# YonghaoHe/LFD-A-Light-and-Fast-Detector

Hardware: AMD Instinct MI355X
Metric: images/sec WIDERFACE-S 1920x1080 bs=8 end-to-end inference, LFD.precision='fp32_storage' (raw logits within 1e-4 of fp32: inside north_star's 1e-3; the 'fp16' mode, sigma 2.5e-3, under fp16_mode) (higher is better)
Workload: dtype f16

## Files before the change

### include/lfd_hip.h

```cpp
#ifndef LFD_HIP_H_
#define LFD_HIP_H_

#include <stddef.h>
#include <stdint.h>

#ifdef __cplusplus
extern "C" {
#endif

#define LFD_HIP_ABI_VERSION 3
#define LFD_MAX_LEVELS 8

typedef void* lfd_stream_t;

#if defined(LFD_BUILDING)
#define LFD_API __attribute__((visibility("default")))
#else
#define LFD_API
#endif

enum lfd_status {
  LFD_OK = 0,
  LFD_ERR_INVALID_ARGUMENT = -1,
  LFD_ERR_WORKSPACE_TOO_SMALL = -2,
// ... 332 lines not shown
  const float* b0;
  const void* w1;
  const float* b1;
  void* gn_sums;
  const void* gn_in_sums;
  const float* gn_in_gamma;
  const float* gn_in_beta;
  float* f_out0;
  float* f_out1;
  const float* scale1;
  int64_t in_plane_halfs;
  int32_t pixels, pad_;
} lfd_pl_head_level_t;
LFD_API int lfd_pl_head_levels(const lfd_pl_head_desc_t* desc, const lfd_pl_head_level_t* levels, int32_t num_levels,
                               const void* zeros, lfd_stream_t stream);

LFD_API int lfd_stem_conv_f16(const void* in, int32_t in_format, int32_t n, int32_t h, int32_t w,
                              int32_t channels, const void* w1_packed, const float* b1,
                              const void* w2_packed, const float* b2, void* out, lfd_stream_t stream);

LFD_API int lfd_stem_gray_f16(const void* in, int32_t in_format, int32_t n, int32_t h, int32_t w, int32_t channels,
                              const void* w1_packed, const float* b1, const void* w2_packed, const float* b2, void* out,
                              lfd_stream_t stream);
LFD_API int lfd_pl_stem_gray_pair(const void* in, int32_t in_format, int32_t n, int32_t h, int32_t w, int32_t channels,
                                  const void* w1_packed, const float* b1, const void* w2_packed, const float* b2, void* out,
                                  int64_t out_plane_halfs, lfd_stream_t stream);

LFD_API int lfd_stem_faster_fused_f16(const void* in, int32_t in_format, int32_t n, int32_t h, int32_t w,
                                      int32_t channels, const void* w1_packed, const float* b1,
                                      const void* w2_packed, const float* b2, const void* w3_packed,
// ... 468 lines not shown
```

### lfd-a-light-and-fast-detector_amd/csrc/planes_head.hip

```cpp
#include "planes_impl.h"

namespace pl {

struct PhLevel {
  const void* in;
  long in_plane;
  float* out;
  const half8* w0;
  const float* b0;
  const half8* w1;
  const float* b1;
  unsigned long long* gn_out;
  const unsigned long long* gn_in;
  const float* gamma;
  const float* beta;
  float* f_out0;
  float* f_out1;
  const float* scale1;
  int P, tiles_per_img, tile_start, pad_;
};
struct PhArgs {
  PhLevel lv[LFD_MAX_LEVELS];
  const _Float16* zeros;
  long w_plane0, w_plane1;
// ... 21 lines not shown
  static_assert(LDS_BYTES <= 80 * 1024, "two workgroups per CU");
};

__device__ __forceinline__ double wave_sum(double v) {
#pragma unroll
  for (int d = 32; d >= 1; d >>= 1) v += __shfl_xor(v, d);
  return v;
}

#ifdef LFD_PL_TIMING
#define PH_T(i) do { if (blockIdx.x == PL_DBG_BLOCK && threadIdx.x == 0 && dbg_it < 8) g_pl_dbg[dbg_it * 16 + (i)] = __builtin_readcyclecounter(); } while (0)
#else
#define PH_T(i)
#endif

template <int MODE, int CIN, int NSLAB>
__global__ __launch_bounds__(256, 2) void k_pl_head(PhArgs a) {
  using C = PhCfg<MODE, CIN, NSLAB>;
  extern __shared__ __attribute__((aligned(16))) char smem[];
  const int lane = threadIdx.x & 63;
  const int wave = __builtin_amdgcn_readfirstlane((int)(threadIdx.x >> 6));
  const int h = lane >> 5, pix = lane & 31;
  constexpr int PT = MODE == 2 ? 1 : 2;
  const int slab = MODE == 2 ? (wave % NSLAB) : wave;
  const int pt0 = MODE == 2 ? (wave / NSLAB) : 0;
  const bool mfma_wave = MODE != 2 || wave < 2 * NSLAB;

  const int nblk = gridDim.x;
  const int xcd = blockIdx.x & 7, bix = blockIdx.x >> 3;
  const int per_xcd = (a.ntiles + 7) / 8;
  const int t_begin = xcd * per_xcd;
  const int t_end = (t_begin + per_xcd) < a.ntiles ? (t_begin + per_xcd) : a.ntiles;
  const int wgs_xcd = (nblk + 7 - xcd) / 8;
#ifdef PH_STRIDED
  const int t_step = wgs_xcd;
  const int t_first = t_begin + bix, t_last = t_end;
#else
  const int t_step = 1;
  const int chunk = (t_end - t_begin + wgs_xcd - 1) / (wgs_xcd > 0 ? wgs_xcd : 1);
  const int t_first = t_begin + bix * chunk;
  const int t_last = (t_first + chunk) < t_end ? (t_first + chunk) : t_end;
#endif
  int lstart[LFD_MAX_LEVELS];
#pragma unroll
  for (int i = 0; i < LFD_MAX_LEVELS; ++i) lstart[i] = i < a.n_levels ? a.lv[i].tile_start : 0x7fffffff;
  auto level_of = [&](int t) {
    int l = 0;
#pragma unroll
    for (int i = 1; i < LFD_MAX_LEVELS; ++i) l += (t >= lstart[i]) ? 1 : 0;
    return l;
  };

  auto with_level = [&](int l, auto&& f) {
    static_for([&](auto ic) {
      constexpr int i = decltype(ic)::value;
      if (l == i) f(a.lv[i]);
    }, std::make_integer_sequence<int, LFD_MAX_LEVELS>{});
// ... 113 lines not shown
  int buf = 0;
  bool first = true;
  if (t < t_last) issue_in(t, 0);

  for (; t < t_last; t += t_step, ++dbg_it) {
    PH_T(0);
    const int l = level_of(t);
    const bool new_level = l != cur_l;
    if (new_level) with_level(l, [&](const PhLevel& v) { lv = v; });
    const int rel = t - lv.tile_start;
    const int n = rel / lv.tiles_per_img;
    const int j = rel - n * lv.tiles_per_img;
    const int p0 = j * C::TPX;
    const bool has_next = t + t_step < t_last;

    if (first) asm volatile("s_waitcnt vmcnt(0)" ::: "memory");
    else if constexpr (MODE != 2) asm volatile("s_waitcnt vmcnt(8)" ::: "memory");
    else {
      switch (n_st) {
        case 0: asm volatile("s_waitcnt vmcnt(0)" ::: "memory"); break;
        case 1: asm volatile("s_waitcnt vmcnt(1)" ::: "memory"); break;
        case 2: asm volatile("s_waitcnt vmcnt(2)" ::: "memory"); break;
        case 3: asm volatile("s_waitcnt vmcnt(3)" ::: "memory"); break;
        case 4: asm volatile("s_waitcnt vmcnt(4)" ::: "memory"); break;
        case 5: asm volatile("s_waitcnt vmcnt(5)" ::: "memory"); break;
        case 6: asm volatile("s_waitcnt vmcnt(6)" ::: "memory"); break;
        case 7: asm volatile("s_waitcnt vmcnt(7)" ::: "memory"); break;
        case 8: asm volatile("s_waitcnt vmcnt(8)" ::: "memory"); break;
        case 9: asm volatile("s_waitcnt vmcnt(9)" ::: "memory"); break;
        case 10: asm volatile("s_waitcnt vmcnt(10)" ::: "memory"); break;
        case 11: asm volatile("s_waitcnt vmcnt(11)" ::: "memory"); break;
// ... 6 lines not shown
    }
    first = false;
    PH_T(1);
    block_barrier();
    PH_T(2);
    if constexpr (PLANES_IN && C::NBUF == 2) {
      if (has_next) issue_in(t + t_step, buf ^ 1);
    }

    if (new_level) {
      cur_l = l;
      const half8* ws = lv.w0 + ((size_t)slab * C::NK0) * 64 + lane;
#pragma unroll
      for (int k = 0; k < C::NK0; ++k) {
        w0h[k] = ws[(size_t)k * 64];
        w0l[k] = ws[a.w_plane0 + (size_t)k * 64];
      }
      if constexpr (MODE == 0) {
        const half8* w1s = lv.w1 + ((size_t)slab * 8) * 64 + lane;
#pragma unroll
        for (int k = 0; k < 8; ++k) {
          w1h[k] = w1s[(size_t)k * 64];
          w1l[k] = w1s[a.w_plane1 + (size_t)k * 64];
        }
      }
      if (threadIdx.x < 128) {
        sbias[threadIdx.x] = (MODE == 2 && (int)threadIdx.x >= NSLAB * 32) ? 0.f : lv.b0[threadIdx.x];
        if constexpr (MODE == 0) sbias[128 + threadIdx.x] = lv.b1[threadIdx.x];
      }
      if constexpr (MODE == 2) {
        n_st = 0;
        if (mfma_wave) {
#pragma unroll
          for (int i = 0; i < 16; ++i) n_st += (slab * 32 + 8 * (i >> 2) + (i & 3) < a.f_c0 + a.f_c1) ? 1 : 0;
        }
      }
      gnin_key = -1;
      block_barrier();
    }

    const char* op = smem + C::OP_OFF;
    if constexpr (!PLANES_IN) {
      const int pj = (int)threadIdx.x & 31, gi = pj >> 1;
      if (gnin_key != n) {
        gnin_key = n;
        long long s = 0, q = 0;
#pragma unroll
        for (int r = 0; r < kGnRep; ++r) {
          s += (long long)lv.gn_in[(((size_t)r * a.N + n) * 16 + gi) * 2];
          q += (long long)lv.gn_in[(((size_t)r * a.N + n) * 16 + gi) * 2 + 1];
        }
        const double cnt = (double)lv.P * 8.0;
        const double m = (double)s / kGnFix / cnt;
        double var = (double)q / kGnFix / cnt - m * m;
        var = var > 0. ? var : 0.;
        const float rstd = (float)(1. / sqrt(var + (double)a.eps)), mean = (float)m;
#pragma unroll
        for (int e = 0; e < 4; ++e) {
          gn_a[e] = rstd * lv.gamma[pj * 4 + e];
          gn_b[e] = lv.beta[pj * 4 + e] - mean * gn_a[e];
        }
      }
      const char* raw = smem + C::IN_OFF;
      char* opw = smem + C::OP_OFF;
#pragma unroll
      for (int r = 0; r < 8; ++r) {
        const int p = ((int)threadIdx.x >> 5) + 8 * r;
        const float4 v = *reinterpret_cast<const float4*>(raw + p * 512 + pj * 16);
        const float y0 = fmaxf(fmaf(v.x, gn_a[0], gn_b[0]), 0.f), y1 = fmaxf(fmaf(v.y, gn_a[1], gn_b[1]), 0.f);
        const float y2 = fmaxf(fmaf(v.z, gn_a[2], gn_b[2]), 0.f), y3 = fmaxf(fmaf(v.w, gn_a[3], gn_b[3]), 0.f);
        uint2 oh, ol;
        split2(y0, y1, oh.x, ol.x);
        split2(y2, y3, oh.y, ol.y);
        const int o = p * 256 + ((gi ^ (p & 15)) * 16) + (pj & 1) * 8;
        *reinterpret_cast<uint2*>(opw + o) = oh;
        *reinterpret_cast<uint2*>(opw + C::OP_PLANE + o) = ol;
      }
      PH_T(3);
      block_barrier();
      PH_T(4);
      if (has_next) issue_in(t + t_step, 0);
      PH_T(5);
// ... 46 lines not shown

    if constexpr (MODE == 0) {
      const char* xb = smem + C::IN_OFF + buf * 2 * C::IN_PLANE;
      init_acc(sbias + slab * 32 + 4 * h);
      contract([&](int q, int pt) { return xb + xi[pt] + (((2 * q) ^ xikey) << 4); }, C::IN_PLANE, w0h, w0l, std::integral_constant<int, C::NK0>{});
      char* mid = smem + C::OP_OFF;
#pragma unroll
      for (int pt = 0; pt < 2; ++pt) {
        const int pb = pt * 32 + pix;
#pragma unroll
        for (int g = 0; g < 4; ++g) {
          float y[4];
#pragma unroll
          for (int e = 0; e < 4; ++e) {
            y[e] = comb(am[pt][4 * g + e], ac[pt][4 * g + e]);
            if (a.relu0) y[e] = fmaxf(y[e], 0.f);
          }
          uint2 vh, vl;
          split2(y[0], y[1], vh.x, vl.x);
          split2(y[2], y[3], vh.y, vl.y);
          const int o = pb * 256 + (((slab * 4 + g) ^ (pb & 15)) * 16) + 8 * h;
          *reinterpret_cast<uint2*>(mid + o) = vh;
          *reinterpret_cast<uint2*>(mid + C::OP_PLANE + o) = vl;
        }
      }
      block_barrier();
      if constexpr (C::NBUF == 1) {
        if (has_next) issue_in(t + t_step, 0);
      }
      init_acc(sbias + 128 + slab * 32 + 4 * h);
      contract([&](int q, int pt) { return op_addr(op, q, pt); }, C::OP_PLANE, w1h, w1l, std::integral_constant<int, 8>{});
// ... 2 lines not shown
      init_acc(sbias + slab * 32 + 4 * h);
      contract([&](int q, int pt) { return xb + xi[pt] + (((2 * q) ^ xikey) << 4); }, C::IN_PLANE, w0h, w0l, std::integral_constant<int, C::NK0>{});
    } else {
      if (mfma_wave) {
        init_acc(sbias + slab * 32 + 4 * h);
        contract([&](int q, int pt) { return op_addr(op, q, pt); }, C::OP_PLANE, w0h, w0l, std::integral_constant<int, 8>{});
      }
    }

    PH_T(6);
    if constexpr (MODE != 2) {
      if (n != gn_n || l != gn_l) {
        gn_flush();
        gn_n = n; gn_l = l; gn_dst = lv.gn_out;
      }
      float* trash = reinterpret_cast<float*>(const_cast<_Float16*>(a.zeros) + 1024) + (threadIdx.x & 127) * 4;
      float* obase = lv.out + ((size_t)n * lv.P + p0) * 128 + slab * 32 + 4 * h;
#pragma unroll
      for (int pt = 0; pt < 2; ++pt) {
        const int px = pt * 32 + pix;
        const bool ok = p0 + px < lv.P;
        float* orow = obase + (size_t)px * 128;
#pragma unroll
        for (int g = 0; g < 4; ++g) {
          float4 v;
          v.x = comb(am[pt][4 * g + 0], ac[pt][4 * g + 0]);
          v.y = comb(am[pt][4 * g + 1], ac[pt][4 * g + 1]);
          v.z = comb(am[pt][4 * g + 2], ac[pt][4 * g + 2]);
          v.w = comb(am[pt][4 * g + 3], ac[pt][4 * g + 3]);
          *reinterpret_cast<float4*>(ok ? orow + 8 * g : trash) = v;
          if (ok) {
            const float s = (v.x + v.y) + (v.z + v.w);
            const float q = fmaf(v.x, v.x, fmaf(v.y, v.y, fmaf(v.z, v.z, v.w * v.w)));
            gs[g] += (double)s;
            gq[g] += (double)q;
          }
        }
      }
    } else {
      if (mfma_wave) {
        const float sc1 = lv.scale1 ? *lv.scale1 : 1.f;
        const int ctot = a.f_c0 + a.f_c1;
        float* trash = reinterpret_cast<float*>(const_cast<_Float16*>(a.zeros) + 1024) + (threadIdx.x & 127);
        const int px = p0 + pt0 * 32 + pix;
        const bool in_img = px < lv.P;
        const size_t pixi = in_img ? (size_t)px : 0;
        float* q0 = lv.f_out0 + (size_t)n * a.f_img0 + pixi * a.f_c0;
        float* q1 = lv.f_out1 + (size_t)n * a.f_img1 + pixi * a.f_c1 - a.f_c0;
#pragma unroll
        for (int g = 0; g < 4; ++g)
#pragma unroll
          for (int e = 0; e < 4; ++e) {
            if (slab * 32 + 8 * g + e < ctot) {
              const int co = slab * 32 + 8 * g + 4 * h + e;
              const float y = comb(am[0][4 * g + e], ac[0][4 * g + e]);
              const bool first_out = co < a.f_c0;
              float* dst = (in_img && co < ctot) ? (first_out ? q0 : q1) + co : trash;
              *dst = first_out ? y : y * sc1;
            }
          }
      }
    }
    if constexpr (PLANES_IN && C::NBUF == 2) buf ^= 1;
    PH_T(7);
  }
  gn_flush();
}

template <int NSLAB>
__global__ __launch_bounds__(256, 2) void k_pl_head_out(PhArgs a) {
  constexpr int TPX = 64, OP_PLANE = TPX * 256, BIAS_OFF = 4 * OP_PLANE;
  extern __shared__ __attribute__((aligned(16))) char smem[];
  const int lane = threadIdx.x & 63;
  const int wave = __builtin_amdgcn_readfirstlane((int)(threadIdx.x >> 6));
  const int h = lane >> 5, pix = lane & 31;
  const int slab = wave % NSLAB, pt0 = wave / NSLAB;
  const bool mfma_wave = wave < 2 * NSLAB;
  const int pj = (int)threadIdx.x & 31, gi = pj >> 1, prow = (int)threadIdx.x >> 5;
  const int nblk = gridDim.x;
  const int xcd = blockIdx.x & 7, bix = blockIdx.x >> 3;
  const int per_xcd = (a.ntiles + 7) / 8;
// ... 448 lines not shown
  static unsigned long long attr_done_mask = 0;
  const int attr_done_dev = lfd_device_ordinal();
  if (LFD_ONCE_PER_DEVICE(attr_done_mask, attr_done_dev)) {
    if (hipFuncSetAttribute(reinterpret_cast<const void*>(kern), hipFuncAttributeMaxDynamicSharedMemorySize, C::LDS_BYTES) != hipSuccess)
      return LFD_ERR_LAUNCH_FAILED;
    LFD_DONE_ON_DEVICE(attr_done_mask, attr_done_dev);
  }
  int blocks = 512;
  if (blocks > 8 * ((a.ntiles + 7) / 8)) blocks = 8 * ((a.ntiles + 7) / 8);
  if (blocks < 1) blocks = 1;
  hipLaunchKernelGGL(kern, dim3(blocks), dim3(256), C::LDS_BYTES, st, a);
  LFD_CHECK_LAUNCH();
  return LFD_OK;
}

}

#ifdef LFD_PL_TIMING
extern "C" __attribute__((visibility("default"))) int lfd_debug_pl_head_timing(unsigned long long* host_out) {
  return (int)hipMemcpyFromSymbol(host_out, HIP_SYMBOL(pl::g_pl_dbg), sizeof(unsigned long long) * 136);
}
#endif

extern "C" int lfd_pl_head_levels(const lfd_pl_head_desc_t* d, const lfd_pl_head_level_t* levels, int32_t num_levels, const void* zeros,
                                  lfd_stream_t stream) {
  hipStream_t st = reinterpret_cast<hipStream_t>(stream);
  if (!d || !levels || !zeros || num_levels < 1 || num_levels > LFD_MAX_LEVELS || d->n < 1) return LFD_ERR_INVALID_ARGUMENT;
  if (d->mode < 0 || d->mode > 3) return LFD_ERR_INVALID_ARGUMENT;
  if (d->mode == 0 && d->cin != 64 && d->cin != 128) return LFD_ERR_UNSUPPORTED;
  if (d->mode == 2 && (d->f_c0 < 0 || d->f_c1 < 0 || d->f_c0 + d->f_c1 < 1 || d->f_c0 + d->f_c1 > 64)) return LFD_ERR_UNSUPPORTED;
  pl::PhArgs a{};
  a.zeros = (const _Float16*)zeros;
  a.n_levels = num_levels; a.N = d->n; a.relu0 = d->relu0; a.eps = d->gn_in_eps;
  a.f_c0 = d->f_c0; a.f_c1 = d->f_c1; a.f_img0 = d->f_image_stride0; a.f_img1 = d->f_image_stride1;
  const int nslab0 = d->mode == 2 ? (d->f_c0 + d->f_c1 + 31) / 32 : 4;
  const int nk0 = (d->mode == 0 ? d->cin : 128) / 16;
  a.w_plane0 = (long)nslab0 * nk0 * 64;
  a.w_plane1 = 4L * 8 * 64;
  for (int i = 0; i < num_levels; ++i) {
    const lfd_pl_head_level_t& s = levels[i];
    if (!s.in || !s.w0 || !s.b0 || s.pixels < 1) return LFD_ERR_INVALID_ARGUMENT;
    if (!lfd_aligned16(s.in) || !lfd_aligned16(s.out) || (s.in_plane_halfs & 7)) return LFD_ERR_INVALID_ARGUMENT;
    if (d->mode == 0 && (!s.w1 || !s.b1)) return LFD_ERR_INVALID_ARGUMENT;
    if (d->mode != 2 && (!s.out || !s.gn_sums)) return LFD_ERR_INVALID_ARGUMENT;
    if ((d->mode == 1 || d->mode == 2) && (!s.gn_in_sums || !s.gn_in_gamma || !s.gn_in_beta)) return LFD_ERR_INVALID_ARGUMENT;
    if (d->mode == 2 && ((d->f_c0 > 0 && !s.f_out0) || (d->f_c1 > 0 && !s.f_out1))) return LFD_ERR_INVALID_ARGUMENT;
    pl::PhLevel& l = a.lv[i];
    l.in = s.in; l.in_plane = s.in_plane_halfs; l.out = (float*)s.out;
    l.w0 = (const half8*)s.w0; l.b0 = s.b0; l.w1 = (const half8*)s.w1; l.b1 = s.b1;
    l.gn_out = (unsigned long long*)s.gn_sums; l.gn_in = (const unsigned long long*)s.gn_in_sums;
    l.gamma = s.gn_in_gamma; l.beta = s.gn_in_beta;
    l.f_out0 = s.f_out0; l.f_out1 = s.f_out1; l.scale1 = s.scale1;
    l.P = s.pixels;
  }
  if (d->mode == 0) return d->cin == 64 ? pl::launch_pl_head<0, 64, 4>(a, st) : pl::launch_pl_head<0, 128, 4>(a, st);
  if (d->mode == 3) return pl::launch_pl_head<3, 128, 4>(a, st);
  if (d->mode == 1) return lfd_tune(LFD_TUNE_PL_HEAD_ROLES) != 0 ? pl::launch_pl_head_b2(a, st) : pl::launch_pl_head<1, 128, 4>(a, st);
  if (lfd_tune(LFD_TUNE_PL_HEAD_OUT_REGS) != 0) return nslab0 == 1 ? pl::launch_pl_head_out<1>(a, st) : pl::launch_pl_head_out<2>(a, st);
  return nslab0 == 1 ? pl::launch_pl_head<2, 128, 1>(a, st) : pl::launch_pl_head<2, 128, 2>(a, st);
}
```

### lfd-a-light-and-fast-detector_amd/lfd_amd/_lib.py

```python
import ctypes as C
import os

_HERE = os.path.dirname(os.path.abspath(__file__))
LIB_PATH = os.environ.get('LFD_HIP_LIB') or os.path.join(_HERE, 'liblfd_hip.so')
MAX_LEVELS = 8
F32, F16 = 0, 1

_lib = None


class DetectDesc(C.Structure):
    _fields_ = [('num_levels', C.c_int32),
                ('level_h', C.c_int32 * MAX_LEVELS), ('level_w', C.c_int32 * MAX_LEVELS),
                ('level_stride', C.c_int32 * MAX_LEVELS),
                ('level_range_lo', C.c_float * MAX_LEVELS), ('level_range_hi', C.c_float * MAX_LEVELS),
                ('num_classes', C.c_int32), ('num_cls_channels', C.c_int32),
                ('score_mode', C.c_int32), ('decode_mode', C.c_int32),
                ('class_agnostic', C.c_int32), ('max_candidates', C.c_int32),
                ('score_thr', C.c_float), ('iou_thr', C.c_float)]


class DetectExt(C.Structure):
    _fields_ = [('pre_nms_limit', C.c_int32), ('post_nms_limit', C.c_int32)]

# ... 57 lines not shown
class PlLevel(C.Structure):
    _fields_ = [(k, C.c_void_p) for k in ('in_', 'out', 'w_packed', 'bias', 'tail_w_packed', 'tail_bias', 'gn_sums', 'gn_in_sums',
                                          'gn_in_gamma', 'gn_in_beta', 'f_out0', 'f_out1', 'scale1')] + \
               [('h', C.c_int32), ('w', C.c_int32), ('in_plane_halfs', C.c_int64), ('out_plane_halfs', C.c_int64)]


class PlHeadDesc(C.Structure):
    _fields_ = [('mode', C.c_int32), ('n', C.c_int32), ('cin', C.c_int32), ('relu0', C.c_int32), ('f_c0', C.c_int32), ('f_c1', C.c_int32),
                ('gn_in_eps', C.c_float), ('pad_', C.c_int32), ('f_image_stride0', C.c_int64), ('f_image_stride1', C.c_int64)]


class PlHeadLevel(C.Structure):
    _fields_ = [(k, C.c_void_p) for k in ('in_', 'out', 'w0', 'b0', 'w1', 'b1', 'gn_sums', 'gn_in_sums', 'gn_in_gamma', 'gn_in_beta',
                                          'f_out0', 'f_out1', 'scale1')] + \
               [('in_plane_halfs', C.c_int64), ('pixels', C.c_int32), ('pad_', C.c_int32)]


PL_GN_REPLICAS = 8
ABI_VERSION = 3
HEAD_FOLDED_HALFS = 4 * 9 * 64 * 8
HEAD_TOWER1_GROUP_HALFS = 8 * 64 * 8


class AssignDesc(C.Structure):
    _fields_ = [('n', C.c_int32), ('num_levels', C.c_int32),
                ('level_h', C.c_int32 * MAX_LEVELS), ('level_w', C.c_int32 * MAX_LEVELS), ('stride', C.c_int32 * MAX_LEVELS),
                ('reg_lo', C.c_int32 * MAX_LEVELS), ('reg_hi', C.c_int32 * MAX_LEVELS),
                ('gray_lo', C.c_int32 * MAX_LEVELS), ('gray_hi', C.c_int32 * MAX_LEVELS),
                ('total_points', C.c_int32), ('num_classes', C.c_int32),
                ('assign_mode', C.c_int32), ('independent', C.c_int32)]
# ... 235 lines not shown
    'lfd_conv_packed_weight_halfs': (_SZ, [_I32, _I32, _I32]),
    'lfd_conv2d_nhwc_f16': (C.c_int, [C.POINTER(ConvDesc), _P, _P, _P, _P, _P, _P, _P, _P, _P]),
    'lfd_fasterblock_fused_f16': (C.c_int, [_I32, _I32, _I32, _P, _P, _P, _P, _P, _P, _P, _P]),
    'lfd_fasterblock128_fused_f16': (C.c_int, [_I32, _I32, _I32, _P, _P, _P, _P, _P, _P, _P]),
    'lfd_downblock_fused_f16': (C.c_int, [_I32, _I32, _I32, _P, _P, _P, _P, _P, _P, _P, _P, _P, _P]),
    'lfd_conv2d_nhwc_f16_acc32': (C.c_int, [C.POINTER(ConvDesc), _P, _P, _P, _P, _P, _P]),
    'lfd_p32_conv_packed_weight_halfs': (_SZ, [_I32, _I32, _I32]),
    'lfd_p32_conv2d_nhwc_f32': (C.c_int, [C.POINTER(P32ConvDesc), _P, _P, _P, _P, _P, _P, _P]),
    'lfd_p32_conv2d_tail_nhwc_f32': (C.c_int, [C.POINTER(P32ConvDesc), _P, _P, _P, _P, _P, _P, _I32, _P]),
    'lfd_pl_stem_pair': (C.c_int, [_P, _I32, _I32, _I32, _I32, _I32, _P, _P, _P, _P, _P, _I64, _P]),
    'lfd_pl_stem2x': (C.c_int, [_P, _I32, _I32, _I32, _I32, _P, _P, _P, _P, _P, _P, _P, _P, _I64, _P, _P]),
    'lfd_pl_conv2d': (C.c_int, [C.POINTER(PlConvDesc), _P, _P, _P, _P, _P, _P, _P, _P, _P, _P, _P, _P, _P, _P, _P, _P, _P, _P, _P]),
    'lfd_pl_block64': (C.c_int, [_I32, _I32, _I32, _P, _I64, _P, _I64, _P, _P, _P, _P, _P, _P]),
    'lfd_pl_conv2d_levels': (C.c_int, [C.POINTER(PlConvDesc), C.POINTER(PlLevel), _I32, _P, _P]),
    'lfd_pl_head_levels': (C.c_int, [C.POINTER(PlHeadDesc), C.POINTER(PlHeadLevel), _I32, _P, _P]),
    'lfd_pl_groupnorm_relu': (C.c_int, [_P, _I64, _I32, _I64, _I32, _P, _P, _P, _F, _I32, _P]),
    'lfd_p32_groupnorm_workspace_bytes': (_SZ, [_I32, _I32]),
    'lfd_p32_groupnorm_relu_f32': (C.c_int, [_P, _I32, _I64, _I32, _I32, _P, _P, _F, _I32, _P, _SZ, _P]),
    'lfd_conv2d_downsample_nhwc_f16': (C.c_int, [C.POINTER(ConvDesc), _P, _P, _P, _P, _P, _P, _P, _P, _P]),
    'lfd_batch_assemble_f32': (C.c_int, [_P, _P, _P, _P, _P, _I32, _I32, _I32, _I32, _I32, _P, _P]),
    'lfd_plan_bbox_crop_batch': (C.c_int, [C.POINTER(PlanDesc), C.POINTER(PlanBufs), _P]),
    'lfd_eval_append_dets_f32': (C.c_int, [C.POINTER(EvalDesc), C.POINTER(EvalBufs), _P, _P, _P, _I32, _I32, _P, _I32, _P, _I32, _P]),
    'lfd_eval_append_rows_f64': (C.c_int, [C.POINTER(EvalDesc), C.POINTER(EvalBufs), _P, _I64, _P, _I32, _P]),
    'lfd_eval_match_workspace_bytes': (_SZ, [C.POINTER(EvalDesc)]),
    'lfd_eval_match': (C.c_int, [C.POINTER(EvalDesc), C.POINTER(EvalBufs), _P, _SZ, _P]),
    'lfd_eval_accumulate_workspace_bytes': (_SZ, [C.POINTER(EvalDesc)]),
    'lfd_eval_accumulate': (C.c_int, [C.POINTER(EvalDesc), C.POINTER(EvalBufs), _P, _SZ, _P]),
    'lfd_eval_tt100k_append_dets_f32': (C.c_int, [C.POINTER(TT100KEvalDesc), C.POINTER(TT100KEvalBufs), _P, _P, _P, _I32, _I32, _P, _I32,
                                                  _P, _P]),
    'lfd_eval_tt100k_append_rows_f64': (C.c_int, [C.POINTER(TT100KEvalDesc), C.POINTER(TT100KEvalBufs), _P, _I64, _P, _I32, _P]),
# ... 68 lines not shown
```

### lfd-a-light-and-fast-detector_amd/lfd_amd/engine_p2.py

```python
import ctypes as C
import os

import torch
import torch.nn as nn

from . import _lib, engine, ops
from ._lib import check, lib, ptr, stream_ptr

_UNION = engine._UNION
_LO = 2048.0


class Unsupported(Exception):
    pass


def _split(w):
    w = w.detach().float()
    hi = w.half()
    lo = ((w - hi.float()) * _LO).half()
    return hi, lo


def pack_planes_weight(w):
# ... 83 lines not shown
}


def _check_dispatch(cin, cout, ks, stride, tail, ds, res, gn, out32):
    opts = _DISPATCH.get((cin, ks, stride, -(-cout // 32)))
    used = {k for k, v in (('tail', tail), ('ds', ds), ('res', res), ('gn', gn), ('out32', out32)) if v}
    if opts is None or not (used - {'gn'} <= opts and (not gn or 'gn' in opts)) or len(used - {'gn'}) > 1:
        raise Unsupported('no plane kernel for conv %d -> %d k%d s%d %s' % (cin, cout, ks, stride, sorted(used)))
    if gn and (res or ds or out32):
        raise Unsupported('GroupNorm sums ride on a plain or chained 1x1')


def _fork_enabled():
    import os
    return os.environ.get('LFD_P2_FORK', '0') != '0'


def _levels_enabled():
    return os.environ.get('LFD_P2_LEVELS', '1') != '0'


class _Op(object):
    __slots__ = ('kind', 'src', 'dst', 'res', 'ds_dst', 'cin', 'cout', 'ks', 'stride', 'relu', 'w', 'b', 'tail', 'ds',
                 'out_mode', 'gn', 'gnin', 'level', 'f_c0', 'f_c1', 'scale', 'w1', 'b1', 'w2', 'b2', 'channels')

    def __init__(self, kind):
        self.kind = kind
        for k in self.__slots__[1:]:
            setattr(self, k, None)

# ... 286 lines not shown
            elif o.tail is None and o.gnin is not None and o.out_mode == 2 and o.cin == 128 and o.f_c0 + o.f_c1 <= 64:
                modes.append(2)
            elif plain and o.gn is not None and o.out_mode == 1 and o.cin == 128 and o.cout == 128:
                modes.append(3)
            elif plain and o.gn is None and o.out_mode == 0:
                modes.append('G')
            else:
                return None
        return modes if any(m != 'G' for m in modes) else None

    def _flat_launches(self, modes):
        launches, made_in = [], {}
        for grp, mode in zip(self.level_groups, modes):
            srcs = [self.ops[i].src for i in grp]
            target = None
            if mode in (1, 3):
                for li in range(len(launches) - 1, -1, -1):
                    m2, ops2 = launches[li]
                    if m2 == mode and len(ops2) + len(grp) <= _lib.MAX_LEVELS and all(made_in.get(b_, -1) < li for b_ in srcs):
                        target = li
                        break
                    if any(made_in.get(b_, -1) >= li for b_ in srcs):
                        break
            if target is None:
                launches.append((mode, list(grp)))
                target = len(launches) - 1
            else:
                launches[target][1].extend(grp)
            for i in grp:
                if self.ops[i].dst is not None:
                    made_in[self.ops[i].dst] = target
        return launches

    def _launch_levels_flat(self, st, modes):
        l, sp = lib(), stream_ptr()
        zeros = ptr(ops.zero_line(self.device))
        if st.flat_calls is None:
            calls = []
            for mode, grp in self._flat_launches(modes):
                if mode == 'G':
                    arr = (_lib.PlLevel * len(grp))()
                    d0 = None
                    for j, i in enumerate(grp):
                        o = self.ops[i]
                        d, src, dst, _, _, _, _ = self._desc(o, st)
                        d0 = d0 or d
                        lv = arr[j]
                        lv.in_, lv.out, lv.w_packed, lv.bias = src.data_ptr(), dst.data_ptr(), o.w.data_ptr(), o.b.data_ptr()
                        lv.h, lv.w, lv.in_plane_halfs, lv.out_plane_halfs = src.shape[2], src.shape[3], d.in_plane_halfs, d.out_plane_halfs
                    calls.append(('G', d0, arr, len(grp)))
                    continue
                arr = (_lib.PlHeadLevel * len(grp))()
                d = _lib.PlHeadDesc()
                for j, i in enumerate(grp):
                    o = self.ops[i]
                    src = st.bufs[o.src]
                    lv, gi = arr[j], o.gnin
                    lv.in_, lv.w0, lv.b0 = src.data_ptr(), o.w.data_ptr(), o.b.data_ptr()
                    lv.pixels, lv.in_plane_halfs = src.shape[2] * src.shape[3], src[0].numel()
                    d.mode, d.n, d.cin, d.relu0 = mode, st.n, o.cin, o.relu
                    if mode == 0:
                        lv.w1, lv.b1 = o.tail[0].data_ptr(), o.tail[1].data_ptr()
                    if mode != 2:
                        lv.out, lv.gn_sums = st.bufs[o.dst].data_ptr(), st.gn_sums[o.gn].data_ptr()
                    if gi is not None:
                        lv.gn_in_sums, lv.gn_in_gamma, lv.gn_in_beta = st.gn_sums[gi[0]].data_ptr(), gi[1].data_ptr(), gi[2].data_ptr()
                        d.gn_in_eps = gi[3]
                    if mode == 2:
                        d.f_c0, d.f_c1 = o.f_c0, o.f_c1
                        d.f_image_stride0, d.f_image_stride1 = st.P * o.f_c0, st.P * 4
                        lv.f_out0 = (st.cls.data_ptr() + st.p_off[o.level] * o.f_c0 * 4) if o.f_c0 else None
                        lv.f_out1 = (st.reg.data_ptr() + st.p_off[o.level] * 4 * 4) if o.f_c1 else None
                        lv.scale1 = o.scale.data_ptr() if o.scale is not None else None
                calls.append((mode, d, arr, len(grp)))
            st.flat_calls = calls
        for mode, d, arr, n in st.flat_calls:
            if mode == 'G':
                check(l.lfd_pl_conv2d_levels(C.byref(d), arr, n, zeros, sp), 'lfd_pl_conv2d_levels')
            else:
                check(l.lfd_pl_head_levels(C.byref(d), arr, n, zeros, sp), 'lfd_pl_head_levels')

    def _launch_levels(self, st):
        modes = self._flat_head_modes() if _flat_head_enabled() else None
        if modes is not None:
            return self._launch_levels_flat(st, modes)
        l, sp = lib(), stream_ptr()
        zeros = ptr(ops.zero_line(self.device))
        if st.level_calls is None:
            calls = []
            for grp in self.level_groups:
                arr = (_lib.PlLevel * len(grp))()
                d0 = None
                for j, i in enumerate(grp):
# ... 96 lines not shown
                    s //= 2
                self.dims[b] = (hh, ww)
            self.sizes = [self.dims[t] for t in plan.taps]
            self.p_off, p = [], 0
            for hh, ww in self.sizes:
                self.p_off.append(p)
                p += hh * ww
            self.P = p
            self.cls = torch.empty((n, p, plan.cls_channels), dtype=torch.float32, device=dev)
            self.reg = torch.empty((n, p, 4), dtype=torch.float32, device=dev)
            self.gn_sums = torch.zeros((max(plan.num_gn, 1), _lib.PL_GN_REPLICAS, n, 16, 2), dtype=torch.int64, device=dev)
            self.side = torch.cuda.Stream(device=dev)
        self.graph = {}
        self.level_calls = None
        self.flat_calls = None
```

Measured before the change: 6515.

## Merge mode-0 head launches with differing cin/relu into one segmented kernel

Adds a mixed head kernel that runs several contiguous segments of mode-0 head levels, with different input channel counts (64/128) and relu flags, inside one launch. A block-wide barrier separates the segments. The Python planner now merges mode-0 groups into shared launches by default, so fewer kernel launches are issued. Kernel arguments are read through the kernarg pointer, and the wait is forced to drain on level changes. The barrier between segments and the idle blocks in smaller segments may cost some overlap.

After: 6566, median of 4. Within noise of the previous version (+0.8%).

```diff
diff --git a/include/lfd_hip.h b/include/lfd_hip.h
--- a/include/lfd_hip.h
+++ b/include/lfd_hip.h
@@ -370,6 +370,29 @@
 } lfd_pl_head_level_t;
 LFD_API int lfd_pl_head_levels(const lfd_pl_head_desc_t* desc, const lfd_pl_head_level_t* levels, int32_t num_levels,
                                const void* zeros, lfd_stream_t stream);
+
+typedef struct lfd_pl_head_level_ex {
+  const void* in;
+  void* out;
+  const void* w0;
+  const float* b0;
+  const void* w1;
+  const float* b1;
+  void* gn_sums;
+  const void* gn_in_sums;
+  const float* gn_in_gamma;
+  const float* gn_in_beta;
+  float* f_out0;
+  float* f_out1;
+  const float* scale1;
+  int64_t in_plane_halfs;
+  int32_t pixels, pad_;
+  int32_t cin, relu0;
+  float gn_in_eps;
+  int32_t pad2_;
+} lfd_pl_head_level_ex_t;
+LFD_API int lfd_pl_head_levels_ex(const lfd_pl_head_desc_t* desc, const lfd_pl_head_level_ex_t* levels, int32_t num_levels,
+                                  const void* zeros, lfd_stream_t stream);
 
 LFD_API int lfd_stem_conv_f16(const void* in, int32_t in_format, int32_t n, int32_t h, int32_t w,
                               int32_t channels, const void* w1_packed, const float* b1,
diff --git a/lfd-a-light-and-fast-detector_amd/csrc/planes_head.hip b/lfd-a-light-and-fast-detector_amd/csrc/planes_head.hip
--- a/lfd-a-light-and-fast-detector_amd/csrc/planes_head.hip
+++ b/lfd-a-light-and-fast-detector_amd/csrc/planes_head.hip
@@ -59,33 +59,40 @@
 #define PH_T(i)
 #endif
 
+struct PhRange { int t_first, t_last, t_step; };
+__device__ __forceinline__ PhRange ph_range(int ntiles, int nblk, int blk) {
+  PhRange r;
+  const int xcd = blk & 7, bix = blk >> 3;
+  const int per_xcd = (ntiles + 7) / 8;
+  const int t_begin = xcd * per_xcd;
+  const int t_end = (t_begin + per_xcd) < ntiles ? (t_begin + per_xcd) : ntiles;
+  const int wgs_xcd = (nblk + 7 - xcd) / 8;
+#ifdef PH_STRIDED
+  r.t_step = wgs_xcd;
+  r.t_first = t_begin + bix; r.t_last = t_end;
+#else
+  r.t_step = 1;
+  const int chunk = (t_end - t_begin + wgs_xcd - 1) / (wgs_xcd > 0 ? wgs_xcd : 1);
+  r.t_first = t_begin + bix * chunk;
+  r.t_last = (r.t_first + chunk) < t_end ? (r.t_first + chunk) : t_end;
+#endif
+  return r;
+}
+
 template <int MODE, int CIN, int NSLAB>
-__global__ __launch_bounds__(256, 2) void k_pl_head(PhArgs a) {
+__device__ __forceinline__ void ph_run(const PhArgs& a, char* smem, const int t_first, const int t_last, const int t_step, const int relu0,
+                                       const long w_plane0) {
   using C = PhCfg<MODE, CIN, NSLAB>;
-  extern __shared__ __attribute__((aligned(16))) char smem[];
-  const int lane = threadIdx.x & 63;
-  const int wave = __builtin_amdgcn_readfirstlane((int)(threadIdx.x >> 6));
+  unsigned tid = threadIdx.x;
+  asm volatile("" : "+v"(tid));
+  const int lane = tid & 63;
+  const int wave = __builtin_amdgcn_readfirstlane((int)(tid >> 6));
   const int h = lane >> 5, pix = lane & 31;
   constexpr int PT = MODE == 2 ? 1 : 2;
   const int slab = MODE == 2 ? (wave % NSLAB) : wave;
   const int pt0 = MODE == 2 ? (wave / NSLAB) : 0;
   const bool mfma_wave = MODE != 2 || wave < 2 * NSLAB;
 
-  const int nblk = gridDim.x;
-  const int xcd = blockIdx.x & 7, bix = blockIdx.x >> 3;
-  const int per_xcd = (a.ntiles + 7) / 8;
-  const int t_begin = xcd * per_xcd;
-  const int t_end = (t_begin + per_xcd) < a.ntiles ? (t_begin + per_xcd) : a.ntiles;
-  const int wgs_xcd = (nblk + 7 - xcd) / 8;
-#ifdef PH_STRIDED
-  const int t_step = wgs_xcd;
-  const int t_first = t_begin + bix, t_last = t_end;
-#else
-  const int t_step = 1;
-  const int chunk = (t_end - t_begin + wgs_xcd - 1) / (wgs_xcd > 0 ? wgs_xcd : 1);
-  const int t_first = t_begin + bix * chunk;
-  const int t_last = (t_first + chunk) < t_end ? (t_first + chunk) : t_end;
-#endif
   int lstart[LFD_MAX_LEVELS];
 #pragma unroll
   for (int i = 0; i < LFD_MAX_LEVELS; ++i) lstart[i] = i < a.n_levels ? a.lv[i].tile_start : 0x7fffffff;
@@ -229,7 +236,7 @@
     const int p0 = j * C::TPX;
     const bool has_next = t + t_step < t_last;
 
-    if (first) asm volatile("s_waitcnt vmcnt(0)" ::: "memory");
+    if (first || new_level) asm volatile("s_waitcnt vmcnt(0)" ::: "memory");
     else if constexpr (MODE != 2) asm volatile("s_waitcnt vmcnt(8)" ::: "memory");
     else {
       switch (n_st) {
@@ -266,7 +273,7 @@
 #pragma unroll
       for (int k = 0; k < C::NK0; ++k) {
         w0h[k] = ws[(size_t)k * 64];
-        w0l[k] = ws[a.w_plane0 + (size_t)k * 64];
+        w0l[k] = ws[w_plane0 + (size_t)k * 64];
       }
       if constexpr (MODE == 0) {
         const half8* w1s = lv.w1 + ((size_t)slab * 8) * 64 + lane;
@@ -276,9 +283,9 @@
           w1l[k] = w1s[a.w_plane1 + (size_t)k * 64];
         }
       }
-      if (threadIdx.x < 128) {
-        sbias[threadIdx.x] = (MODE == 2 && (int)threadIdx.x >= NSLAB * 32) ? 0.f : lv.b0[threadIdx.x];
-        if constexpr (MODE == 0) sbias[128 + threadIdx.x] = lv.b1[threadIdx.x];
+      if (tid < 128) {
+        sbias[tid] = (MODE == 2 && (int)tid >= NSLAB * 32) ? 0.f : lv.b0[tid];
+        if constexpr (MODE == 0) sbias[128 + tid] = lv.b1[tid];
       }
       if constexpr (MODE == 2) {
         n_st = 0;
@@ -293,7 +300,7 @@
 
     const char* op = smem + C::OP_OFF;
     if constexpr (!PLANES_IN) {
-      const int pj = (int)threadIdx.x & 31, gi = pj >> 1;
+      const int pj = (int)tid & 31, gi = pj >> 1;
       if (gnin_key != n) {
         gnin_key = n;
         long long s = 0, q = 0;
@@ -317,7 +324,7 @@
       char* opw = smem + C::OP_OFF;
 #pragma unroll
       for (int r = 0; r < 8; ++r) {
-        const int p = ((int)threadIdx.x >> 5) + 8 * r;
+        const int p = ((int)tid >> 5) + 8 * r;
         const float4 v = *reinterpret_cast<const float4*>(raw + p * 512 + pj * 16);
         const float y0 = fmaxf(fmaf(v.x, gn_a[0], gn_b[0]), 0.f), y1 = fmaxf(fmaf(v.y, gn_a[1], gn_b[1]), 0.f);
         const float y2 = fmaxf(fmaf(v.z, gn_a[2], gn_b[2]), 0.f), y3 = fmaxf(fmaf(v.w, gn_a[3], gn_b[3]), 0.f);
@@ -394,7 +401,7 @@
 #pragma unroll
           for (int e = 0; e < 4; ++e) {
             y[e] = comb(am[pt][4 * g + e], ac[pt][4 * g + e]);
-            if (a.relu0) y[e] = fmaxf(y[e], 0.f);
+            if (relu0) y[e] = fmaxf(y[e], 0.f);
           }
           uint2 vh, vl;
           split2(y[0], y[1], vh.x, vl.x);
@@ -427,7 +434,7 @@
         gn_flush();
         gn_n = n; gn_l = l; gn_dst = lv.gn_out;
       }
-      float* trash = reinterpret_cast<float*>(const_cast<_Float16*>(a.zeros) + 1024) + (threadIdx.x & 127) * 4;
+      float* trash = reinterpret_cast<float*>(const_cast<_Float16*>(a.zeros) + 1024) + (tid & 127) * 4;
       float* obase = lv.out + ((size_t)n * lv.P + p0) * 128 + slab * 32 + 4 * h;
 #pragma unroll
       for (int pt = 0; pt < 2; ++pt) {
@@ -454,7 +461,7 @@
       if (mfma_wave) {
         const float sc1 = lv.scale1 ? *lv.scale1 : 1.f;
         const int ctot = a.f_c0 + a.f_c1;
-        float* trash = reinterpret_cast<float*>(const_cast<_Float16*>(a.zeros) + 1024) + (threadIdx.x & 127);
+        float* trash = reinterpret_cast<float*>(const_cast<_Float16*>(a.zeros) + 1024) + (tid & 127);
         const int px = p0 + pt0 * 32 + pix;
         const bool in_img = px < lv.P;
         const size_t pixi = in_img ? (size_t)px : 0;
@@ -478,6 +485,50 @@
     PH_T(7);
   }
   gn_flush();
+}
+
+template <class T>
+__device__ __forceinline__ const T* ph_kernarg() {
+  return (const T*)__builtin_amdgcn_kernarg_segment_ptr();
+}
+
+template <int MODE, int CIN, int NSLAB>
+__global__ __launch_bounds__(256, 2) void k_pl_head(PhArgs a) {
+  extern __shared__ __attribute__((aligned(16))) char smem[];
+  const PhArgs& ka = *ph_kernarg<PhArgs>();
+  (void)a;
+  const PhRange r = ph_range(ka.ntiles, (int)gridDim.x, (int)blockIdx.x);
+  ph_run<MODE, CIN, NSLAB>(ka, smem, r.t_first, r.t_last, r.t_step, ka.relu0, ka.w_plane0);
+}
+
+struct PhSeg {
+  int t_begin, ntiles, nblk, cin, relu0;
+};
+struct PhMixArgs {
+  PhArgs a;
+  PhSeg seg[LFD_MAX_LEVELS];
+  int n_seg;
+};
+
+__global__ __launch_bounds__(256, 2) void k_pl_head_mix(PhMixArgs m) {
+  static_assert(PhCfg<0, 64, 4>::LDS_BYTES == PhCfg<0, 128, 4>::LDS_BYTES && PhCfg<0, 64, 4>::OP_OFF == PhCfg<0, 128, 4>::OP_OFF,
+                "one LDS layout serves both bodies");
+  extern __shared__ __attribute__((aligned(16))) char smem[];
+  const PhMixArgs& km = *ph_kernarg<PhMixArgs>();
+  (void)m;
+#pragma nounroll
+  for (int s = 0; s < km.n_seg; ++s) {
+    int t_begin = 0, ntiles = 0, nblk = 0, cin = 0, relu0 = 0;
+    static_for([&](auto ic) {
+      constexpr int i = decltype(ic)::value;
+      if (s == i) { t_begin = km.seg[i].t_begin; ntiles = km.seg[i].ntiles; nblk = km.seg[i].nblk; cin = km.seg[i].cin; relu0 = km.seg[i].relu0; }
+    }, std::make_integer_sequence<int, LFD_MAX_LEVELS>{});
+    if (s > 0) block_barrier();
+    if ((int)blockIdx.x >= nblk) continue;
+    const PhRange r = ph_range(ntiles, nblk, (int)blockIdx.x);
+    if (cin == 64) ph_run<0, 64, 4>(km.a, smem, t_begin + r.t_first, t_begin + r.t_last, r.t_step, relu0, 4L * 4 * 64);
+    else ph_run<0, 128, 4>(km.a, smem, t_begin + r.t_first, t_begin + r.t_last, r.t_step, relu0, 4L * 8 * 64);
+  }
 }
 
 template <int NSLAB>
@@ -956,6 +1007,62 @@
   return LFD_OK;
 }
 
+int launch_pl_head_mix(PhMixArgs& m, const int* cin, const int* relu0, hipStream_t st) {
+  using C = PhCfg<0, 64, 4>;
+  PhArgs& a = m.a;
+  long nt = 0;
+  int blocks = 1;
+  m.n_seg = 0;
+  for (int i = 0; i < a.n_levels; ++i) {
+    a.lv[i].tiles_per_img = (a.lv[i].P + C::TPX - 1) / C::TPX;
+    a.lv[i].tile_start = (int)nt;
+    const long lt = (long)a.N * a.lv[i].tiles_per_img;
+    nt += lt;
+    if (nt > 0x7fffffffL) return LFD_ERR_UNSUPPORTED;
+    if (m.n_seg == 0 || m.seg[m.n_seg - 1].cin != cin[i] || m.seg[m.n_seg - 1].relu0 != relu0[i]) {
+      PhSeg& sg = m.seg[m.n_seg++];
+      sg.t_begin = a.lv[i].tile_start; sg.ntiles = 0; sg.cin = cin[i]; sg.relu0 = relu0[i];
+    }
+    m.seg[m.n_seg - 1].ntiles += (int)lt;
+  }
+  a.ntiles = (int)nt;
+  for (int s = 0; s < m.n_seg; ++s) {
+    int b = 512;
+    if (b > 8 * ((m.seg[s].ntiles + 7) / 8)) b = 8 * ((m.seg[s].ntiles + 7) / 8);
+    if (b < 1) b = 1;
+    m.seg[s].nblk = b;
+    if (b > blocks) blocks = b;
+  }
+  auto kern = k_pl_head_mix;
+  static unsigned long long attr_done_mask = 0;
+  const int attr_done_dev = lfd_device_ordinal();
+  if (LFD_ONCE_PER_DEVICE(attr_done_mask, attr_done_dev)) {
+    if (hipFuncSetAttribute(reinterpret_cast<const void*>(kern), hipFuncAttributeMaxDynamicSharedMemorySize, C::LDS_BYTES) != hipSuccess)
+      return LFD_ERR_LAUNCH_FAILED;
+    LFD_DONE_ON_DEVICE(attr_done_mask, attr_done_dev);
+  }
+  hipLaunchKernelGGL(kern, dim3(blocks), dim3(256), C::LDS_BYTES, st, m);
+  LFD_CHECK_LAUNCH();
+  return LFD_OK;
+}
+
+template <class L>
+int ph_fill_level(int mode, int f_c0, int f_c1, const L& s, PhLevel& l) {
+  if (!s.in || !s.w0 || !s.b0 || s.pixels < 1) return LFD_ERR_INVALID_ARGUMENT;
+  if (!lfd_aligned16(s.in) || !lfd_aligned16(s.out) || (s.in_plane_halfs & 7)) return LFD_ERR_INVALID_ARGUMENT;
+  if (mode == 0 && (!s.w1 || !s.b1)) return LFD_ERR_INVALID_ARGUMENT;
+  if (mode != 2 && (!s.out || !s.gn_sums)) return LFD_ERR_INVALID_ARGUMENT;
+  if ((mode == 1 || mode == 2) && (!s.gn_in_sums || !s.gn_in_gamma || !s.gn_in_beta)) return LFD_ERR_INVALID_ARGUMENT;
+  if (mode == 2 && ((f_c0 > 0 && !s.f_out0) || (f_c1 > 0 && !s.f_out1))) return LFD_ERR_INVALID_ARGUMENT;
+  l.in = s.in; l.in_plane = s.in_plane_halfs; l.out = (float*)s.out;
+  l.w0 = (const half8*)s.w0; l.b0 = s.b0; l.w1 = (const half8*)s.w1; l.b1 = s.b1;
+  l.gn_out = (unsigned long long*)s.gn_sums; l.gn_in = (const unsigned long long*)s.gn_in_sums;
+  l.gamma = s.gn_in_gamma; l.beta = s.gn_in_beta;
+  l.f_out0 = s.f_out0; l.f_out1 = s.f_out1; l.scale1 = s.scale1;
+  l.P = s.pixels;
+  return LFD_OK;
+}
+
 }
 
 #ifdef LFD_PL_TIMING
@@ -980,20 +1087,8 @@
   a.w_plane0 = (long)nslab0 * nk0 * 64;
   a.w_plane1 = 4L * 8 * 64;
   for (int i = 0; i < num_levels; ++i) {
-    const lfd_pl_head_level_t& s = levels[i];
-    if (!s.in || !s.w0 || !s.b0 || s.pixels < 1) return LFD_ERR_INVALID_ARGUMENT;
-    if (!lfd_aligned16(s.in) || !lfd_aligned16(s.out) || (s.in_plane_halfs & 7)) return LFD_ERR_INVALID_ARGUMENT;
-    if (d->mode == 0 && (!s.w1 || !s.b1)) return LFD_ERR_INVALID_ARGUMENT;
-    if (d->mode != 2 && (!s.out || !s.gn_sums)) return LFD_ERR_INVALID_ARGUMENT;
-    if ((d->mode == 1 || d->mode == 2) && (!s.gn_in_sums || !s.gn_in_gamma || !s.gn_in_beta)) return LFD_ERR_INVALID_ARGUMENT;
-    if (d->mode == 2 && ((d->f_c0 > 0 && !s.f_out0) || (d->f_c1 > 0 && !s.f_out1))) return LFD_ERR_INVALID_ARGUMENT;
-    pl::PhLevel& l = a.lv[i];
-    l.in = s.in; l.in_plane = s.in_plane_halfs; l.out = (float*)s.out;
-    l.w0 = (const half8*)s.w0; l.b0 = s.b0; l.w1 = (const half8*)s.w1; l.b1 = s.b1;
-    l.gn_out = (unsigned long long*)s.gn_sums; l.gn_in = (const unsigned long long*)s.gn_in_sums;
-    l.gamma = s.gn_in_gamma; l.beta = s.gn_in_beta;
-    l.f_out0 = s.f_out0; l.f_out1 = s.f_out1; l.scale1 = s.scale1;
-    l.P = s.pixels;
+    const int rc = pl::ph_fill_level(d->mode, d->f_c0, d->f_c1, levels[i], a.lv[i]);
+    if (rc != LFD_OK) return rc;
   }
   if (d->mode == 0) return d->cin == 64 ? pl::launch_pl_head<0, 64, 4>(a, st) : pl::launch_pl_head<0, 128, 4>(a, st);
   if (d->mode == 3) return pl::launch_pl_head<3, 128, 4>(a, st);
@@ -1001,3 +1096,24 @@
   if (lfd_tune(LFD_TUNE_PL_HEAD_OUT_REGS) != 0) return nslab0 == 1 ? pl::launch_pl_head_out<1>(a, st) : pl::launch_pl_head_out<2>(a, st);
   return nslab0 == 1 ? pl::launch_pl_head<2, 128, 1>(a, st) : pl::launch_pl_head<2, 128, 2>(a, st);
 }
+
+extern "C" int lfd_pl_head_levels_ex(const lfd_pl_head_desc_t* d, const lfd_pl_head_level_ex_t* levels, int32_t num_levels, const void* zeros,
+                                     lfd_stream_t stream) {
+  hipStream_t st = reinterpret_cast<hipStream_t>(stream);
+  if (!d || !levels || !zeros || num_levels < 1 || num_levels > LFD_MAX_LEVELS || d->n < 1) return LFD_ERR_INVALID_ARGUMENT;
+  if (d->mode < 0 || d->mode > 3) return LFD_ERR_INVALID_ARGUMENT;
+  if (d->mode != 0) return LFD_ERR_UNSUPPORTED;
+  pl::PhMixArgs m{};
+  pl::PhArgs& a = m.a;
+  a.zeros = (const _Float16*)zeros;
+  a.n_levels = num_levels; a.N = d->n;
+  a.w_plane1 = 4L * 8 * 64;
+  int cin[LFD_MAX_LEVELS], relu0[LFD_MAX_LEVELS];
+  for (int i = 0; i < num_levels; ++i) {
+    if (levels[i].cin != 64 && levels[i].cin != 128) return LFD_ERR_UNSUPPORTED;
+    const int rc = pl::ph_fill_level(0, 0, 0, levels[i], a.lv[i]);
+    if (rc != LFD_OK) return rc;
+    cin[i] = levels[i].cin; relu0[i] = levels[i].relu0 != 0;
+  }
+  return pl::launch_pl_head_mix(m, cin, relu0, st);
+}
diff --git a/lfd-a-light-and-fast-detector_amd/lfd_amd/_lib.py b/lfd-a-light-and-fast-detector_amd/lfd_amd/_lib.py
--- a/lfd-a-light-and-fast-detector_amd/lfd_amd/_lib.py
+++ b/lfd-a-light-and-fast-detector_amd/lfd_amd/_lib.py
@@ -95,6 +95,10 @@
     _fields_ = [(k, C.c_void_p) for k in ('in_', 'out', 'w0', 'b0', 'w1', 'b1', 'gn_sums', 'gn_in_sums', 'gn_in_gamma', 'gn_in_beta',
                                           'f_out0', 'f_out1', 'scale1')] + \
                [('in_plane_halfs', C.c_int64), ('pixels', C.c_int32), ('pad_', C.c_int32)]
+
+
+class PlHeadLevelEx(C.Structure):
+    _fields_ = PlHeadLevel._fields_ + [('cin', C.c_int32), ('relu0', C.c_int32), ('gn_in_eps', C.c_float), ('pad2_', C.c_int32)]
 
 
 PL_GN_REPLICAS = 8
@@ -360,6 +364,7 @@
     'lfd_pl_block64': (C.c_int, [_I32, _I32, _I32, _P, _I64, _P, _I64, _P, _P, _P, _P, _P, _P]),
     'lfd_pl_conv2d_levels': (C.c_int, [C.POINTER(PlConvDesc), C.POINTER(PlLevel), _I32, _P, _P]),
     'lfd_pl_head_levels': (C.c_int, [C.POINTER(PlHeadDesc), C.POINTER(PlHeadLevel), _I32, _P, _P]),
+    'lfd_pl_head_levels_ex': (C.c_int, [C.POINTER(PlHeadDesc), C.POINTER(PlHeadLevelEx), _I32, _P, _P]),
     'lfd_pl_groupnorm_relu': (C.c_int, [_P, _I64, _I32, _I64, _I32, _P, _P, _P, _F, _I32, _P]),
     'lfd_p32_groupnorm_workspace_bytes': (_SZ, [_I32, _I32]),
     'lfd_p32_groupnorm_relu_f32': (C.c_int, [_P, _I32, _I64, _I32, _I32, _P, _P, _F, _I32, _P, _SZ, _P]),
diff --git a/lfd-a-light-and-fast-detector_amd/lfd_amd/engine_p2.py b/lfd-a-light-and-fast-detector_amd/lfd_amd/engine_p2.py
--- a/lfd-a-light-and-fast-detector_amd/lfd_amd/engine_p2.py
+++ b/lfd-a-light-and-fast-detector_amd/lfd_amd/engine_p2.py
@@ -121,6 +121,11 @@
 def _fork_enabled():
     import os
     return os.environ.get('LFD_P2_FORK', '0') != '0'
+
+
+def _head_merge_enabled():
+    import os
+    return os.environ.get('LFD_P2_HEADMERGE', '1') != '0'
 
 
 def _levels_enabled():
@@ -437,7 +442,7 @@
         for grp, mode in zip(self.level_groups, modes):
             srcs = [self.ops[i].src for i in grp]
             target = None
-            if mode in (1, 3):
+            if mode in (1, 3) or (mode == 0 and _head_merge_enabled()):
                 for li in range(len(launches) - 1, -1, -1):
                     m2, ops2 = launches[li]
                     if m2 == mode and len(ops2) + len(grp) <= _lib.MAX_LEVELS and all(made_in.get(b_, -1) < li for b_ in srcs):
@@ -453,12 +458,23 @@
             for i in grp:
                 if self.ops[i].dst is not None:
                     made_in[self.ops[i].dst] = target
+        for mode, ops_ in launches:
+            if mode != 'G' and not self._per_level_fields(mode):
+                sigs = set((self.ops[i].cin, bool(self.ops[i].relu), self.ops[i].gnin[3] if self.ops[i].gnin is not None else None)
+                           for i in ops_)
+                if len(sigs) != 1:
+                    raise ValueError('flat head launch of mode %s merges ops that differ in (cin, relu, eps): %s' % (mode, sorted(sigs, key=repr)))
         return launches
+
+    @staticmethod
+    def _per_level_fields(mode):
+        return mode == 0 and _head_merge_enabled()
 
     def _launch_levels_flat(self, st, modes):
         l, sp = lib(), stream_ptr()
         zeros = ptr(ops.zero_line(self.device))
-        if st.flat_calls is None:
+        if st.flat_calls is None or st.flat_calls_merge != _head_merge_enabled():
+            st.flat_calls_merge = _head_merge_enabled()
             calls = []
             for mode, grp in self._flat_launches(modes):
                 if mode == 'G':
@@ -473,12 +489,15 @@
                         lv.h, lv.w, lv.in_plane_halfs, lv.out_plane_halfs = src.shape[2], src.shape[3], d.in_plane_halfs, d.out_plane_halfs
                     calls.append(('G', d0, arr, len(grp)))
                     continue
-                arr = (_lib.PlHeadLevel * len(grp))()
+                ex = self._per_level_fields(mode)
+                arr = ((_lib.PlHeadLevelEx if ex else _lib.PlHeadLevel) * len(grp))()
                 d = _lib.PlHeadDesc()
                 for j, i in enumerate(grp):
                     o = self.ops[i]
                     src = st.bufs[o.src]
                     lv, gi = arr[j], o.gnin
+                    if ex:
+                        lv.cin, lv.relu0, lv.gn_in_eps = o.cin, o.relu, gi[3] if gi is not None else 0.0
                     lv.in_, lv.w0, lv.b0 = src.data_ptr(), o.w.data_ptr(), o.b.data_ptr()
                     lv.pixels, lv.in_plane_halfs = src.shape[2] * src.shape[3], src[0].numel()
                     d.mode, d.n, d.cin, d.relu0 = mode, st.n, o.cin, o.relu
@@ -495,11 +514,13 @@
                         lv.f_out0 = (st.cls.data_ptr() + st.p_off[o.level] * o.f_c0 * 4) if o.f_c0 else None
                         lv.f_out1 = (st.reg.data_ptr() + st.p_off[o.level] * 4 * 4) if o.f_c1 else None
                         lv.scale1 = o.scale.data_ptr() if o.scale is not None else None
-                calls.append((mode, d, arr, len(grp)))
+                calls.append(('X' if ex else mode, d, arr, len(grp)))
             st.flat_calls = calls
         for mode, d, arr, n in st.flat_calls:
             if mode == 'G':
                 check(l.lfd_pl_conv2d_levels(C.byref(d), arr, n, zeros, sp), 'lfd_pl_conv2d_levels')
+            elif mode == 'X':
+                check(l.lfd_pl_head_levels_ex(C.byref(d), arr, n, zeros, sp), 'lfd_pl_head_levels_ex')
             else:
                 check(l.lfd_pl_head_levels(C.byref(d), arr, n, zeros, sp), 'lfd_pl_head_levels')
 
@@ -626,3 +647,4 @@
         self.graph = {}
         self.level_calls = None
         self.flat_calls = None
+        self.flat_calls_merge = None
```
